# hellojialee/Improved-Body-Parts

Hardware: NVIDIA H100
Metric: grouping images/sec @128x128 heatmaps, 30 persons/img (higher is better)
Workload: dtype f32 body-part maps, f32 keypoint maps; f64 coordinates/scores

## Files before the change

improved_body_parts_b200/csrc/common.cuh:

```cuda
#pragma once

#include <cuda_runtime.h>
#include <stdint.h>

#include <algorithm>

namespace spg {

#ifdef SPG_TRACE
constexpr int kTraceCtas = 64, kTraceSlots = 1024;
__device__ unsigned long long g_spg_trace[kTraceCtas * kTraceSlots];
__device__ __forceinline__ void trace_put(int slot, int dep, bool value_only) {
    if (blockIdx.x < kTraceCtas && (threadIdx.x & 31) == 0) {
        unsigned long long t;
        asm volatile("mov.u64 %0, %%clock64;" : "=l"(t) : "r"(dep) : "memory");
        g_spg_trace[blockIdx.x * kTraceSlots + slot] = value_only ? (unsigned long long)(unsigned)dep : t;
    }
}
#define SPG_TR(slot, dep) ::spg::trace_put((slot), (int)(dep), false)
#define SPG_TRV(slot, v) ::spg::trace_put((slot), (int)(v), true)
#else
#define SPG_TR(slot, dep) do {} while (0)
#define SPG_TRV(slot, v) do {} while (0)
#endif

constexpr int kMaxParts = 32;
constexpr int kMaxLimbs = 64;
constexpr int kMaxCapPeaks = 128;
constexpr int kMaxCapRows = 128;
constexpr int kMaxRefineRadius = 4;
constexpr int kMaxOutJoints = 32;

constexpr uint32_t kStPeakOverflow = 1u << 0;
constexpr uint32_t kStCandOverflow = 1u << 1;
constexpr uint32_t kStRowOverflow = 1u << 2;
constexpr uint32_t kStSampleIndex = 1u << 3;
constexpr uint32_t kStAssert = 1u << 4;
constexpr uint32_t kStWireOverflow = 1u << 5;

struct Params {
    double thre1, thre2, connect_ration, len_rate, connection_tole, min_mean_score;
    int32_t mid_num, offset_radius, remove_recon, min_parts;
    int32_t crit1_strict, refresh_len_check;
};

struct Workspace {
    int K, L, J, capP, capC, capR, max_batch;
    int16_t limbs[kMaxLimbs * 2];
    int16_t out_from_part[kMaxOutJoints];
    double *peak_x, *peak_y;
    float *peak_score;
    uint32_t *peak_anchor;
    int32_t *peak_count;
    double *cand_prio, *cand_score;
    uint32_t *cand_ij;
    unsigned long long *cand_key;
    int32_t *cand_count;
    int32_t *surv_count;
    uint32_t *conn_ij;
    double *conn_score, *conn_norm;
    int32_t *conn_count;
    double *subset;
    int32_t *n_persons;
    double *people_xy;
    double *people_score;
    uint32_t *status;
    unsigned char *wire;
    long long wire_first;
    int wire_rows;
};

__device__ __forceinline__ uint32_t smem_u32(const void *p) { return (uint32_t)__cvta_generic_to_shared(p); }

__device__ __forceinline__ void mbar_init(uint64_t *bar, uint32_t count) {
    asm volatile("mbarrier.init.shared::cta.b64 [%0], %1;" ::"r"(smem_u32(bar)), "r"(count) : "memory");
}
__device__ __forceinline__ void fence_mbar_init() { asm volatile("fence.mbarrier_init.release.cluster;" ::: "memory"); }
__device__ __forceinline__ void fence_proxy_async() { asm volatile("fence.proxy.async.shared::cta;" ::: "memory"); }
__device__ __forceinline__ void mbar_expect_tx(uint64_t *bar, uint32_t bytes) {
    asm volatile("mbarrier.arrive.expect_tx.shared::cta.b64 _, [%0], %1;" ::"r"(smem_u32(bar)), "r"(bytes) : "memory");
}
__device__ __forceinline__ void bulk_g2s(void *dst_smem, const void *src_gmem, uint32_t bytes, uint64_t *bar) {
    asm volatile("cp.async.bulk.shared::cluster.global.mbarrier::complete_tx::bytes [%0], [%1], %2, [%3];" ::"r"(
                     smem_u32(dst_smem)),
                 "l"(src_gmem), "r"(bytes), "r"(smem_u32(bar))
                 : "memory");
}
__device__ __forceinline__ void mbar_arrive(uint64_t *bar) {
    asm volatile("mbarrier.arrive.shared::cta.b64 _, [%0];" ::"r"(smem_u32(bar)) : "memory");
}
__device__ __forceinline__ bool mbar_try_wait(uint64_t *bar, uint32_t parity) {
    uint32_t ok;
    asm volatile(
        "{\n"
        " .reg .pred p;\n"
        " mbarrier.try_wait.parity.shared::cta.b64 p, [%1], %2;\n"
        " selp.u32 %0, 1, 0, p;\n"
        "}\n"
        : "=r"(ok)
        : "r"(smem_u32(bar)), "r"(parity)
        : "memory");
    return ok != 0;
}
__device__ __forceinline__ void mbar_wait(uint64_t *bar, uint32_t parity) {
    while (!mbar_try_wait(bar, parity)) {
    }
}
__device__ __forceinline__ void mbar_wait_sleep(uint64_t *bar, uint32_t parity, uint32_t hint_ns = 20000u) {
    uint32_t ok = 0;
    while (!ok) {
        asm volatile(
            "{\n"
            " .reg .pred p;\n"
            " mbarrier.try_wait.parity.shared::cta.b64 p, [%1], %2, %3;\n"
            " selp.u32 %0, 1, 0, p;\n"
            "}\n"
            : "=r"(ok)
            : "r"(smem_u32(bar)), "r"(parity), "r"(hint_ns)
            : "memory");
    }
}

template <typename T>
__device__ __forceinline__ T pairwise_sum(const T *a, int n) {
    if (n < 8) {
        T res = (T)0;
        for (int i = 0; i < n; i++) res = res + a[i];
        return res;
    }
    T r[8];
#pragma unroll
    for (int k = 0; k < 8; k++) r[k] = a[k];
    int i = 8;
    for (; i < n - (n % 8); i += 8) {
#pragma unroll
        for (int k = 0; k < 8; k++) r[k] = r[k] + a[i + k];
    }
    T res = ((r[0] + r[1]) + (r[2] + r[3])) + ((r[4] + r[5]) + (r[6] + r[7]));
    for (; i < n; i++) res = res + a[i];
    return res;
}

}
```

improved_body_parts_b200/csrc/limb_score.cuh:

```cuda
#pragma once

#include "common.cuh"

namespace spg {

struct ScoreArgs {
    const void *paf;
    int64_t img_stride, chan_stride;
    int H, W, image_base, mid_num, screen;
    int crit1_strict;
    int exact_warps;
    double image_extent, thre2, connect_ration;
    Workspace ws;
};

constexpr int kScoreThreads = 512;
constexpr uint32_t kBulkChunkBytes = 32768;
constexpr int kScreenMaxMid = 63;
#ifndef SPG_SCREEN_SAMPLES
#define SPG_SCREEN_SAMPLES 10
#endif
constexpr int kScreenSamples = SPG_SCREEN_SAMPLES;
constexpr int kScreenMaxDim = 2048;

struct alignas(8) ScreenTab {
    float inv;
    signed char maxfail;
    unsigned char qn;
    unsigned char pad[2];
};

__host__ __device__ constexpr size_t screen_tables_bytes() {
    return (((size_t)(kScreenMaxMid + 1) * (sizeof(double) + sizeof(ScreenTab) + kScreenSamples * sizeof(float))) + 15) & ~(size_t)15;
}

__device__ __forceinline__ void build_screen_row(const ScoreArgs &a, int m, double *rcp, ScreenTab *tab, float *ts) {
    const double need = __dmul_rn(a.connect_ration, (double)m);
    int need_i = (int)need;
    if ((double)need_i < need || (a.crit1_strict && (double)need_i == need)) need_i++;
    rcp[m] = m > 0 ? __ddiv_rn(1.0, (double)m) : 0.0;
    const int lo = m / 8, hi = m - 1 - lo;
    const int qn = max(0, min(kScreenSamples, hi - lo + 1));
    for (int q = 0; q < kScreenSamples; q++)
        ts[m * kScreenSamples + q] = (float)(qn > 1 ? lo + (min(q, qn - 1) * (hi - lo)) / (qn - 1) : lo);
    ScreenTab t;
    t.inv = m > 1 ? 1.0f / (float)(m - 1) : 0.0f;
    t.maxfail = (signed char)max(min(m - need_i, 127), -1);
    t.qn = (unsigned char)qn;
    t.pad[0] = t.pad[1] = 0;
    tab[m] = t;
}

inline size_t score_smem_bytes(size_t plane_bytes, int capP) {
    const size_t plane = (plane_bytes + 127) & ~(size_t)127;
    const size_t peaks = (size_t)capP * (4 * sizeof(double) + 6 * sizeof(float) + 2);
    const size_t words = ((size_t)capP * capP + 31) / 32;
    return plane + ((peaks + 15) & ~(size_t)15) + screen_tables_bytes() + words * (sizeof(uint32_t) + sizeof(uint16_t)) + 16;
}

__device__ __forceinline__ bool inside_map(double x, double y, int H, int W) {
    return x >= 0.0 && x <= (double)(W - 1) && y >= 0.0 && y <= (double)(H - 1);
}

struct PairGeom {
    const double *ax, *ay, *bx, *by;
    const float *as, *bs;
    const double *rcp;
};

template <typename T, int kExactBatch = 1, typename TA = T>
__device__ __forceinline__ bool score_pair_exact(const T *__restrict__ plane, int H, int W, const ScoreArgs &a,
                                                 const PairGeom &g, int i, int j, bool interior, TA thre2,
                                                 double &score, double &prio, bool &bad) {
    const double ax = g.ax[i], ay = g.ay[i], bx = g.bx[j], by = g.by[j];
    const double vx = __dsub_rn(bx, ax), vy = __dsub_rn(by, ay);
    const double n2 = __dadd_rn(__dmul_rn(vx, vx), __dmul_rn(vy, vy));
    if (n2 == 0.0) return false;
    const double half = __dmul_rn(0.5, a.image_extent);
    const double Md = (double)a.mid_num;
    double norm = 0.0;
    int m = a.mid_num;
    const bool need_norm = n2 < __dmul_rn(Md, Md) || n2 > __dmul_rn(__dmul_rn(half, half), 1.0 - 1e-9);
    if (need_norm) {
        norm = __dsqrt_rn(n2);
        m = min(__double2int_rn(__dadd_rn(norm, 1.0)), a.mid_num);
    }
    double stepx = 0.0, stepy = 0.0;
    if (m > 1) {
        const double dd = (double)(m - 1);
        if (m - 1 <= kScreenMaxMid) {
            const double y = g.rcp[m - 1];
            const double qx = __dmul_rn(vx, y), qy = __dmul_rn(vy, y);
            stepx = __fma_rn(__fma_rn(-qx, dd, vx), y, qx);
            stepy = __fma_rn(__fma_rn(-qy, dd, vy), y, qy);
        } else {
            stepx = __ddiv_rn(vx, dd);
            stepy = __ddiv_rn(vy, dd);
        }
    }
    TA sum = (TA)0;
    int above = 0;
    if (interior) {
        const int last = m - 1;
        double td = 0.0;
        if constexpr (kExactBatch <= 1) {
#pragma unroll 4
            for (int t = 0; t < last; t++) {
                const int xi = __double2loint(__dadd_rn(__dadd_rn(__dmul_rn(td, stepx), ax), 6755399441055744.0));
                const int yi = __double2loint(__dadd_rn(__dadd_rn(__dmul_rn(td, stepy), ay), 6755399441055744.0));
                const TA v = (TA)plane[yi * W + xi];
                sum = sum + v;
                above += v > thre2;
                td = __dadd_rn(td, 1.0);
            }
        } else {
            for (int t0 = 0; t0 < last; t0 += kExactBatch) {
                T vv[kExactBatch > 0 ? kExactBatch : 1];
#pragma unroll
                for (int u = 0; u < kExactBatch; u++) {
                    const double tdu = t0 + u < last ? __dadd_rn(td, (double)u) : 0.0;
                    const int xi = __double2loint(__dadd_rn(__dadd_rn(__dmul_rn(tdu, stepx), ax), 6755399441055744.0));
                    const int yi = __double2loint(__dadd_rn(__dadd_rn(__dmul_rn(tdu, stepy), ay), 6755399441055744.0));
                    vv[u] = plane[yi * W + xi];
                }
#pragma unroll
                for (int u = 0; u < kExactBatch; u++) {
                    if (t0 + u < last) {
                        sum = sum + (TA)vv[u];
                        above += (TA)vv[u] > thre2;
                    }
                }
                td = __dadd_rn(td, (double)kExactBatch);
            }
        }
        const TA v = (TA)(m > 1 ? plane[__double2int_rn(by) * W + __double2int_rn(bx)]
                               : plane[__double2int_rn(ay) * W + __double2int_rn(ax)]);
        sum = sum + v;
        above += v > thre2;
    } else {
        for (int t = 0; t < m; t++) {
            double sx, sy;
            if (t == m - 1 && m > 1) {
                sx = bx;
                sy = by;
            } else {
                sx = __dadd_rn(__dmul_rn((double)t, stepx), ax);
                sy = __dadd_rn(__dmul_rn((double)t, stepy), ay);
            }
            int yi = __double2int_rn(sy), xi = __double2int_rn(sx);
            if (yi < 0) yi += H;
            if (xi < 0) xi += W;
            if (yi < 0 || yi >= H || xi < 0 || xi >= W) {
                bad = true;
                return false;
            }
            const TA v = (TA)plane[(size_t)yi * W + xi];
            sum = sum + v;
            above += v > thre2;
        }
    }
    double prior = 0.0;
    if (need_norm && norm > half) prior = __dsub_rn(__ddiv_rn(half, norm), 1.0);
    if (sizeof(TA) == 4) {
        float s = __fdiv_rn((float)sum, (float)m);
        s = __fadd_rn(s, prior < 0.0 ? __double2float_rn(prior) : 0.0f);
        const float pr = __fadd_rn(__fadd_rn(__fmul_rn(0.5f, s), __fmul_rn(0.25f, g.as[i])), __fmul_rn(0.25f, g.bs[j]));
        score = (double)s;
        prio = (double)pr;
    } else {
        score = __dadd_rn(__ddiv_rn((double)sum, (double)m), prior < 0.0 ? prior : 0.0);
        prio = __dadd_rn(__dadd_rn(__dmul_rn(0.5, score), (double)__fmul_rn(0.25f, g.as[i])),
                         (double)__fmul_rn(0.25f, g.bs[j]));
    }
    const double need = __dmul_rn(a.connect_ration, (double)m);
    const bool crit1 = a.crit1_strict ? (double)above > need : (double)above >= need;
    const bool crit2 = score > 0.0;
    return crit1 && crit2;
}

template <typename TA>
__device__ __forceinline__ void store_candidate(const Workspace &ws, size_t out_base, int pos, int i, int j, double score, double prio) {
    const uint32_t ij = ((uint32_t)i << 16) | (uint32_t)j;
    ws.cand_prio[out_base + pos] = prio;
    ws.cand_score[out_base + pos] = score;
    ws.cand_ij[out_base + pos] = ij;
    if (sizeof(TA) == 4) {
        const uint32_t b = __float_as_uint((float)prio);
        const uint32_t ord = (b & 0x80000000u) ? ~b : (b | 0x80000000u);
        ws.cand_key[out_base + pos] = ((unsigned long long)ord << 32) | (unsigned long long)(~ij);
    }
}

__device__ __forceinline__ void publish_limb(const Workspace &ws, int n, size_t slot, int ncand, int nsurv, uint32_t flags) {
    ws.cand_count[slot] = min(ncand, ws.capC);
    if (ws.surv_count) ws.surv_count[slot] = nsurv;
    if (ncand > ws.capC) flags |= kStCandOverflow;
    if (flags) atomicOr(&ws.status[n], flags);
}

__host__ __device__ inline float f32_not_above(double t) {
    float f = (float)t;
    if ((double)f > t) f = nextafterf(f, -INFINITY);
    return f;
}

template <typename T, bool STAGE, typename TA = T>
__global__ void __launch_bounds__(kScoreThreads, 3) limb_score_kernel(ScoreArgs a) {
    extern __shared__ __align__(128) unsigned char smem_raw[];
    __shared__ uint64_t bar;
    __shared__ int s_count;
    __shared__ uint32_t s_flags;
    __shared__ int s_total_surv;
    __shared__ uint32_t s_magic;

    const Workspace &ws = a.ws;
    const int tid = threadIdx.x, lane = tid & 31, warp = tid >> 5;
    const int k = blockIdx.x % ws.L;
    const int n_local = blockIdx.x / ws.L;
    const int n = a.image_base + n_local;
    const int H = a.H, W = a.W, capP = ws.capP;
    const T *gplane = reinterpret_cast<const T *>(a.paf) + (int64_t)n_local * a.img_stride + (int64_t)k * a.chan_stride;
    const size_t plane_bytes = (size_t)H * W * sizeof(T);
    if (tid == 0) {
        s_count = 0;
        s_flags = 0;
        if (STAGE) {
            mbar_init(&bar, 1);
            fence_mbar_init();
            mbar_expect_tx(&bar, (uint32_t)plane_bytes);
            for (size_t off = 0; off < plane_bytes; off += kBulkChunkBytes) {
                const uint32_t bytes = (uint32_t)min((size_t)kBulkChunkBytes, plane_bytes - off);
                bulk_g2s(smem_raw + off, reinterpret_cast<const unsigned char *>(gplane) + off, bytes, &bar);
            }
        }
    }
    const int pa = ws.limbs[2 * k], pb = ws.limbs[2 * k + 1];
    const int nA = min(ws.peak_count[(size_t)n * ws.K + pa], capP);
    const int nB = min(ws.peak_count[(size_t)n * ws.K + pb], capP);
    const size_t slot = (size_t)n * ws.L + k;
    if (nA == 0 || nB == 0) {
        if (tid == 0) {
            ws.cand_count[slot] = -1;
            if (STAGE) mbar_wait(&bar, 0);
        }
        return;
    }

    unsigned char *after = smem_raw + (STAGE ? ((plane_bytes + 127) & ~(size_t)127) : 0);
    double *s_ax = reinterpret_cast<double *>(after);
    double *s_ay = s_ax + capP;
    double *s_bx = s_ay + capP;
    double *s_by = s_bx + capP;
    float *s_as = reinterpret_cast<float *>(s_by + capP);
    float *s_bs = s_as + capP;
    float *s_fax = s_bs + capP;
    float *s_fay = s_fax + capP;
    float *s_fbx = s_fay + capP;
    float *s_fby = s_fbx + capP;
    unsigned char *s_ain = reinterpret_cast<unsigned char *>(s_fby + capP);
    unsigned char *s_bin = s_ain + capP;
    const size_t peaks_bytes = ((size_t)capP * (4 * sizeof(double) + 6 * sizeof(float) + 2) + 15) & ~(size_t)15;
    double *s_rcp = reinterpret_cast<double *>(after + peaks_bytes);
    ScreenTab *s_tab = reinterpret_cast<ScreenTab *>(s_rcp + (kScreenMaxMid + 1));
    float *s_ts = reinterpret_cast<float *>(s_tab + (kScreenMaxMid + 1));
    uint32_t *s_mask = reinterpret_cast<uint32_t *>(after + peaks_bytes + screen_tables_bytes());
    const int npairs = nA * nB;
    const int nwords = (npairs + 31) >> 5;
    uint16_t *s_prefix = reinterpret_cast<uint16_t *>(s_mask + (((size_t)capP * capP + 31) >> 5));

    const size_t baseA = ((size_t)n * ws.K + pa) * capP, baseB = ((size_t)n * ws.K + pb) * capP;
    const bool screen = a.screen && a.mid_num <= kScreenMaxMid && H <= kScreenMaxDim && W <= kScreenMaxDim;
    if (warp == 0) {
        for (int i = lane; i < nA; i += 32) {
            const double x = ws.peak_x[baseA + i], y = ws.peak_y[baseA + i];
            s_ax[i] = x; s_ay[i] = y;
            s_fax[i] = (float)(x * 64.0); s_fay[i] = (float)(y * 64.0);
            s_as[i] = ws.peak_score[baseA + i];
            s_ain[i] = inside_map(x, y, H, W);
        }
    } else if (warp == 1) {
        for (int j = lane; j < nB; j += 32) {
            const double x = ws.peak_x[baseB + j], y = ws.peak_y[baseB + j];
            s_bx[j] = x; s_by[j] = y;
            s_fbx[j] = (float)(x * 64.0); s_fby[j] = (float)(y * 64.0);
            s_bs[j] = ws.peak_score[baseB + j];
            s_bin[j] = inside_map(x, y, H, W);
        }
    } else if (warp < 4) {
        const int m = tid - 64;
        if (m <= a.mid_num && m <= kScreenMaxMid) build_screen_row(a, m, s_rcp, s_tab, s_ts);
        if (tid == 64 + 63) s_magic = nB > 1 ? 0xffffffffu / (uint32_t)nB + 1u : 0u;
    }
    __syncthreads();
    if (STAGE) mbar_wait(&bar, 0);
    const T *plane = STAGE ? reinterpret_cast<const T *>(smem_raw) : gplane;
    const T thre2 = (sizeof(T) == 4 && sizeof(TA) == 8) ? (T)f32_not_above(a.thre2) : (T)a.thre2;
    const TA thre2_exact = (TA)a.thre2;

    const uint32_t magic = s_magic;
    for (int base = 0; base < npairs; base += kScoreThreads) {
        const int p = base + tid;
        bool keep = false;
        if (p < npairs) {
            keep = true;
            if (screen) {
                const int i = nB > 1 ? (int)__umulhi((uint32_t)p, magic) : p;
                const int j = p - i * nB;
                if (s_ain[i] && s_bin[j]) {
                    const float ax64 = s_fax[i], ay64 = s_fay[i];
                    const float dx64 = s_fbx[j] - ax64, dy64 = s_fby[j] - ay64;
                    const float n2 = (dx64 * dx64 + dy64 * dy64) * (1.0f / 4096.0f);
                    if (n2 > 1e-6f) {
                        const float q = n2 * rsqrtf(n2) + 1.0f;
                        const float r = rintf(q);
                        const bool longp = q >= (float)a.mid_num + 0.51f;
                        int m = longp ? a.mid_num : min((int)r, a.mid_num);
                        if (!longp && !(fabsf(q - r) < 0.49f)) m = -1;
                        asm volatile("" : "+r"(m));
                        if (m >= 1) {
                            const ScreenTab tb = s_tab[m];
                            const int maxfail = tb.maxfail;
                            const int qn = tb.qn;
                            const float inv = tb.inv;
                            const float sx64 = dx64 * inv, sy64 = dy64 * inv;
                            const float *ts = s_ts + m * kScreenSamples;
                            int fails = 0;
                            for (int q2 = 0; q2 < qn; q2++) {
                                const float tf = ts[q2];
                                const int xs = __float2int_rn(__fmaf_rn(tf, sx64, ax64));
                                const int ys = __float2int_rn(__fmaf_rn(tf, sy64, ay64));
                                const unsigned cx = (unsigned)(xs + 33) & 63u, cy = (unsigned)(ys + 33) & 63u;
                                const T v = plane[((ys + 32) >> 6) * W + ((xs + 32) >> 6)];
                                fails += (min(cx, cy) > 2u) && !(v > thre2);
                            }
                            keep = fails <= maxfail;
                        }
                    }
                }
            }
        }
        const uint32_t bits = __ballot_sync(0xffffffffu, keep);
        if (lane == 0 && (base >> 5) + warp < nwords) s_mask[(base >> 5) + warp] = bits;
    }
    __syncthreads();
    if (warp == 0) {
        int running = 0;
        for (int w0 = 0; w0 < nwords; w0 += 32) {
            const int w = w0 + lane;
            const int c = w < nwords ? __popc(s_mask[w]) : 0;
            int incl = c;
#pragma unroll
            for (int d = 1; d < 32; d <<= 1) {
                const int o = __shfl_up_sync(0xffffffffu, incl, d);
                if (lane >= d) incl += o;
            }
            if (w < nwords) s_prefix[w] = (uint16_t)(running + incl - c);
            running += __shfl_sync(0xffffffffu, incl, 31);
        }
        if (lane == 0) s_total_surv = running;
    }
    __syncthreads();

    const int total_surv = s_total_surv;
    PairGeom g{s_ax, s_ay, s_bx, s_by, s_as, s_bs, s_rcp};
    const size_t out_base = slot * ws.capC;
    for (int sidx = tid; sidx < total_surv; sidx += kScoreThreads) {
        int lo = 0, hi = nwords - 1;
        while (lo < hi) {
            const int mid = (lo + hi + 1) >> 1;
            if ((int)s_prefix[mid] <= sidx) lo = mid; else hi = mid - 1;
        }
        const int bit = __fns(s_mask[lo], 0, sidx - (int)s_prefix[lo] + 1);
        const int p = (lo << 5) + bit;
        const int i = nB > 1 ? (int)__umulhi((uint32_t)p, magic) : p;
        const int j = p - i * nB;
        double score, prio;
        bool bad = false;
        const bool ok = score_pair_exact<T, 1, TA>(plane, H, W, a, g, i, j, s_ain[i] && s_bin[j], thre2_exact, score, prio, bad);
        if (bad) atomicOr(&s_flags, kStSampleIndex);
        if (ok) {
            const int pos = atomicAdd(&s_count, 1);
            if (pos < ws.capC) store_candidate<TA>(ws, out_base, pos, i, j, score, prio);
        }
    }
    __syncthreads();
    if (tid == 0) publish_limb(ws, n, slot, s_count, total_surv, s_flags);
}

}
```

improved_body_parts_b200/csrc/limb_score_persist.cuh:

```cuda
#pragma once

#include "limb_score.cuh"

namespace spg {

constexpr int kPersistThreads = 1024;
constexpr int kPersistSlots = 3;
constexpr int kMetaSlots = 5;
constexpr int kWorkerWarps = kPersistThreads / 32 - 1;
constexpr int kPersistMaxCapP = 64;
constexpr int kScreenTailBypass = 4;
constexpr int kPersistListCap = 1024;

struct PersistHdr {
    int nA, nB, npairs, n, k, special;
    uint32_t magic;
    int pad;
};

struct alignas(16) PeakSlot {
    double ax[kPersistMaxCapP], ay[kPersistMaxCapP], bx[kPersistMaxCapP], by[kPersistMaxCapP];
    float as[kPersistMaxCapP], bs[kPersistMaxCapP];
    float2 fa[kPersistMaxCapP], fb[kPersistMaxCapP];
    unsigned char ain[kPersistMaxCapP], bin[kPersistMaxCapP];
};

struct alignas(16) MetaSlot {
    PeakSlot peaks;
    uint16_t list[kPersistListCap];
    PersistHdr hdr;
    int nsurv, ncand, bnext;
    uint32_t flags;
};

constexpr size_t kPersistPlaneOffset = (screen_tables_bytes() + kMetaSlots * sizeof(MetaSlot) + 127) & ~(size_t)127;
inline size_t persist_smem_bytes(size_t plane_bytes, int ) {
    const size_t plane = (plane_bytes + 127) & ~(size_t)127;
    return kPersistPlaneOffset + kPersistSlots * plane + 128;
}

constexpr uint32_t kScreenBias = 0x4B400000u >> 6;

struct ScreenCtx {
    const PeakSlot *ps;
    uint32_t base;
    const ScreenTab *tab;
    const float *ts;
    int W, mid_num, nB;
    uint32_t magic;
    float thre2;
};

__device__ __forceinline__ void screen_pair(const ScreenCtx &c, int pc, bool valid, int &fails, int &qn, int &maxfail) {
    const int i = c.nB > 1 ? (int)__umulhi((uint32_t)pc, c.magic) : pc;
    const int jj = pc - i * c.nB;
    const float2 fa = c.ps->fa[i], fb = c.ps->fb[jj];
    const float dx64 = fb.x - fa.x, dy64 = fb.y - fa.y;
    const float n2 = (dx64 * dx64 + dy64 * dy64) * (1.0f / 4096.0f);
    float rs;
    asm("rsqrt.approx.ftz.f32 %0, %1;" : "=f"(rs) : "f"(n2));
    const float qf = n2 * rs + 1.0f;
    const float r = rintf(qf);
    const bool longp = qf >= (float)c.mid_num + 0.51f;
    int m = longp ? c.mid_num : min((int)r, c.mid_num);
    if (!longp && !(fabsf(qf - r) < 0.49f)) m = 0;
    if (!(n2 > 1e-6f) || !valid || fminf(fa.x, fb.x) < 0.0f) m = 0;
    m = max(m, 0);
    const ScreenTab tb = c.tab[m];
    qn = tb.qn;
    maxfail = tb.maxfail;
    const float sx64 = dx64 * tb.inv, sy64 = dy64 * tb.inv;
    const float ax64o = fa.x + 33.0f, ay64o = fa.y + 33.0f;
    const float *ts = c.ts + m * kScreenSamples;
    const int qmax = __reduce_max_sync(0xffffffffu, qn);
    const uint32_t base = c.base;
    fails = 0;
    auto sample = [&](int q2) {
        const float tf = ts[q2];
        const uint32_t xb = __float_as_uint(__fadd_rn(__fmaf_rn(tf, sx64, ax64o), 12582912.0f));
        const uint32_t yb = __float_as_uint(__fadd_rn(__fmaf_rn(tf, sy64, ay64o), 12582912.0f));
        float v;
        asm("ld.shared.f32 %0, [%1];" : "=f"(v) : "r"(base + 4u * ((yb >> 6) * (uint32_t)c.W + (xb >> 6))));
        fails += (int)(min(xb & 63u, yb & 63u) > 2u) & (int)!(v > c.thre2);
    };
    if (qmax == kScreenSamples) {
#pragma unroll
        for (int q2 = 0; q2 < kScreenSamples; q2++) sample(q2);
    } else {
#pragma unroll
        for (int q2 = 0; q2 < kScreenSamples; q2++) {
            if (q2 >= qmax) break;
            sample(q2);
        }
    }
    maxfail += qmax - qn;
}

template <typename TA>
__global__ void __launch_bounds__(kPersistThreads, 1) limb_score_persist_kernel(ScoreArgs a, int n_items) {
    extern __shared__ __align__(128) unsigned char smem_raw[];
    __shared__ uint64_t bar_full[kPersistSlots], bar_screened[kMetaSlots], bar_mfree[kMetaSlots];
    __shared__ uint32_t s_bias_bytes;

    using T = float;
    const Workspace &ws = a.ws;
    const int tid = threadIdx.x, lane = tid & 31, warp = tid >> 5;
    const int H = a.H, W = a.W, capP = ws.capP, L = ws.L;
    const size_t plane_bytes = (size_t)H * W * sizeof(T);
    const size_t plane_stride = (plane_bytes + 127) & ~(size_t)127;
    double *s_rcp = reinterpret_cast<double *>(smem_raw);
    ScreenTab *s_tab = reinterpret_cast<ScreenTab *>(s_rcp + (kScreenMaxMid + 1));
    float *s_ts = reinterpret_cast<float *>(s_tab + (kScreenMaxMid + 1));
    MetaSlot *s_meta = reinterpret_cast<MetaSlot *>(smem_raw + screen_tables_bytes());
    unsigned char *s_planes = smem_raw + kPersistPlaneOffset;
    const int nE = min(max(a.exact_warps, 1), kWorkerWarps - 1), nS = kWorkerWarps - nE;

    if (tid == 0) {
        for (int s = 0; s < kPersistSlots; s++) {
            mbar_init(&bar_full[s], 2);
        }
        for (int e = 0; e < kMetaSlots; e++) {
            mbar_init(&bar_screened[e], nS);
            mbar_init(&bar_mfree[e], nE);
            s_meta[e].nsurv = 0; s_meta[e].ncand = 0; s_meta[e].bnext = 0; s_meta[e].flags = 0;
        }
        s_bias_bytes = 4u * kScreenBias * (uint32_t)(W + 1);
        fence_mbar_init();
    }
    if (tid >= 32 && tid < 32 + kScreenMaxMid + 1) build_screen_row(a, tid - 32, s_rcp, s_tab, s_ts);
    __syncthreads();

    const int G = gridDim.x;
    const int nj = ((int)blockIdx.x < n_items) ? (n_items - 1 - (int)blockIdx.x) / G + 1 : 0;
    const bool screen = a.screen && a.mid_num <= kScreenMaxMid && H <= kScreenMaxDim && W <= kScreenMaxDim;
    const T thre2 = sizeof(TA) == 8 ? f32_not_above(a.thre2) : (T)a.thre2;
    const TA thre2_exact = (TA)a.thre2;
    auto plane_of = [&](int n_local, int k) {
        return reinterpret_cast<const T *>(a.paf) + (int64_t)n_local * a.img_stride + (int64_t)k * a.chan_stride;
    };

    if (warp == 0) {
        constexpr int kMaxE = kPersistMaxCapP / 32;
        double r_xa[kMaxE], r_ya[kMaxE], r_xb[kMaxE], r_yb[kMaxE];
        float r_sa[kMaxE], r_sb[kMaxE];
        int r_cntA = 0, r_cntB = 0;
        auto fetch = [&](int j) {
            const int item = (int)blockIdx.x + j * G;
            const int n_local = item / L, k = item - n_local * L;
            const int n = a.image_base + n_local;
            const int pa = ws.limbs[2 * k], pb = ws.limbs[2 * k + 1];
            r_cntA = ws.peak_count[(size_t)n * ws.K + pa];
            r_cntB = ws.peak_count[(size_t)n * ws.K + pb];
            const size_t baseA = ((size_t)n * ws.K + pa) * capP, baseB = ((size_t)n * ws.K + pb) * capP;
#pragma unroll
            for (int u = 0; u < kMaxE; u++) {
                const int e = lane + 32 * u;
                if (e < capP) {
                    r_xa[u] = ws.peak_x[baseA + e]; r_ya[u] = ws.peak_y[baseA + e];
                    r_xb[u] = ws.peak_x[baseB + e]; r_yb[u] = ws.peak_y[baseB + e];
                    r_sa[u] = ws.peak_score[baseA + e]; r_sb[u] = ws.peak_score[baseB + e];
                }
            }
        };
        auto close_item = [&](int jp) {
            if (lane == 0) {
                MetaSlot &ms = s_meta[jp % kMetaSlots];
                publish_limb(ws, ms.hdr.n, (size_t)ms.hdr.n * L + ms.hdr.k, ms.hdr.special ? -1 : ms.ncand, ms.nsurv, ms.flags);
                ms.nsurv = 0; ms.ncand = 0; ms.bnext = 0; ms.flags = 0;
            }
            __syncwarp();
        };
        if (nj > 0) fetch(0);
        for (int j = 0; j < nj; j++) {
            const int s = j % kPersistSlots, e = j % kMetaSlots;
            if (j >= kPersistSlots) {
                const int jp = j - kPersistSlots;
                mbar_wait_sleep(&bar_screened[jp % kMetaSlots], (jp / kMetaSlots) & 1);
            }
            const int item = (int)blockIdx.x + j * G;
            const int n_local = item / L, k = item - n_local * L;
            const int n = a.image_base + n_local;
            if (lane == 0) {
                const unsigned char *gplane = reinterpret_cast<const unsigned char *>(plane_of(n_local, k));
                unsigned char *dst = s_planes + s * plane_stride;
                mbar_expect_tx(&bar_full[s], (uint32_t)plane_bytes);
                for (size_t off = 0; off < plane_bytes; off += kBulkChunkBytes) {
                    const uint32_t bytes = (uint32_t)min((size_t)kBulkChunkBytes, plane_bytes - off);
                    bulk_g2s(dst + off, gplane + off, bytes, &bar_full[s]);
                }
            }
            if (j >= kMetaSlots) {
                mbar_wait_sleep(&bar_mfree[e], ((j / kMetaSlots) - 1) & 1);
                close_item(j - kMetaSlots);
            }
            MetaSlot &ms = s_meta[e];
            PeakSlot &ps = ms.peaks;
#pragma unroll
            for (int u = 0; u < kMaxE; u++) {
                const int q = lane + 32 * u;
                if (q < capP) {
                    const double xa = r_xa[u], ya = r_ya[u], xb = r_xb[u], yb = r_yb[u];
                    ps.ax[q] = xa; ps.ay[q] = ya; ps.bx[q] = xb; ps.by[q] = yb;
                    ps.as[q] = r_sa[u]; ps.bs[q] = r_sb[u];
                    const bool ain = inside_map(xa, ya, H, W), bin = inside_map(xb, yb, H, W);
                    ps.fa[q] = ain ? make_float2((float)(xa * 64.0), (float)(ya * 64.0)) : make_float2(-1.0f, 0.0f);
                    ps.fb[q] = bin ? make_float2((float)(xb * 64.0), (float)(yb * 64.0)) : make_float2(-1.0f, 0.0f);
                    ps.ain[q] = ain;
                    ps.bin[q] = bin;
                }
            }
            const int nA = min(r_cntA, capP), nB = min(r_cntB, capP);
            const bool special = nA == 0 || nB == 0;
            if (lane == 0) {
                PersistHdr h;
                h.nA = nA; h.nB = nB; h.npairs = special ? 0 : nA * nB; h.n = n; h.k = k; h.special = special;
                h.magic = nB > 1 ? 0xffffffffu / (uint32_t)nB + 1u : 0u;
                h.pad = 0;
                ms.hdr = h;
            }
            __syncwarp();
            if (lane == 0) mbar_arrive(&bar_full[s]);
            if (j + 1 < nj) fetch(j + 1);
        }
        for (int jp = max(0, nj - kMetaSlots); jp < nj; jp++) {
            mbar_wait_sleep(&bar_mfree[jp % kMetaSlots], (jp / kMetaSlots) & 1);
            close_item(jp);
        }
    } else {
        auto exact_one = [&](MetaSlot &ms, const T *plane, int p) {
            const PersistHdr &h = ms.hdr;
            const PeakSlot &ps = ms.peaks;
            const int nB = h.nB;
            const int i = nB > 1 ? (int)__umulhi((uint32_t)p, h.magic) : p;
            const int jj = p - i * nB;
            PairGeom g{ps.ax, ps.ay, ps.bx, ps.by, ps.as, ps.bs, s_rcp};
            double score, prio;
            bool bad = false;
            const bool ok = score_pair_exact<T, 10, TA>(plane, H, W, a, g, i, jj, ps.ain[i] && ps.bin[jj], thre2_exact, score, prio, bad);
            if (bad) atomicOr(&ms.flags, kStSampleIndex);
            if (ok) {
                const size_t out_base = ((size_t)h.n * L + h.k) * ws.capC;
                const int pos = atomicAdd(&ms.ncand, 1);
                if (pos < ws.capC) store_candidate<TA>(ws, out_base, pos, i, jj, score, prio);
            }
        };

        if (warp <= nS) {
            int c0 = warp - 1;
            for (int j = 0; j < nj; j++) {
                const int s = j % kPersistSlots, e = j % kMetaSlots;
                mbar_wait_sleep(&bar_full[s], (j / kPersistSlots) & 1);
                MetaSlot &ms = s_meta[e];
                const int npairs = ms.hdr.npairs;
                if (c0 * 32 < npairs) {
                    const T *plane = reinterpret_cast<const T *>(s_planes + s * plane_stride);
                    const ScreenCtx sc{&ms.peaks, smem_u32(plane) - *(volatile uint32_t *)&s_bias_bytes, s_tab, s_ts, W, a.mid_num,
                                       ms.hdr.nB, ms.hdr.magic, thre2};
                    for (int c = c0; c * 32 < npairs; c += nS) {
                        const int p = c * 32 + lane;
                        bool keep = p < npairs;
                        if (screen && npairs - c * 32 > kScreenTailBypass) {
                            int fails, qn, maxfail;
                            screen_pair(sc, min(p, npairs - 1), keep, fails, qn, maxfail);
                            if (qn > 0) keep = fails <= maxfail;
                        }
                        const uint32_t km = __ballot_sync(0xffffffffu, keep);
                        if (km) {
                            int at = 0;
                            if (lane == 0) at = atomicAdd(&ms.nsurv, __popc(km));
                            at = __shfl_sync(0xffffffffu, at, 0);
                            if (keep) {
                                const int at_me = at + __popc(km & ((1u << lane) - 1u));
                                if (at_me < kPersistListCap) ms.list[at_me] = (uint16_t)p;
                                else exact_one(ms, plane, p);
                            }
                        }
                    }
                }
                __syncwarp();
                if (lane == 0) mbar_arrive(&bar_screened[e]);
                if (++c0 == nS) c0 = 0;
            }
        } else {
            for (int j = 0; j < nj; j++) {
                const int e = j % kMetaSlots;
                mbar_wait_sleep(&bar_screened[e], (j / kMetaSlots) & 1);
                MetaSlot &ms = s_meta[e];
                const int ns = min(ms.nsurv, kPersistListCap);
                if (ns > 0) {
                    const T *gplane = plane_of(ms.hdr.n - a.image_base, ms.hdr.k);
                    for (;;) {
                        if (*(volatile int *)&ms.bnext * 32 >= ns) break;
                        int c = 0;
                        if (lane == 0) c = atomicAdd(&ms.bnext, 1);
                        c = __shfl_sync(0xffffffffu, c, 0);
                        if (c * 32 >= ns) break;
                        const int t = c * 32 + lane;
                        if (t < ns) exact_one(ms, gplane, ms.list[t]);
                        __syncwarp();
                    }
                }
                __syncwarp();
                if (lane == 0) mbar_arrive(&bar_mfree[e]);
            }
        }
    }
}

}
```

improved_body_parts_b200/csrc/spgroup.cu:

```cuda
#include "../../include/spgroup.h"

#include <cuda_runtime.h>

#include <algorithm>
#include <cstdarg>
#include <cstdio>
#include <cstdlib>
#include <cstring>
#include <new>
#include <string>
#include <vector>

#include "assemble.cuh"
#include "common.cuh"
#include "limb_match.cuh"
#include "limb_score.cuh"
#include "limb_score_persist.cuh"
#include "match_assemble.cuh"
#include "nms_peaks.cuh"
#include "nms_peaks_persist.cuh"
#include "nms_peaks_banded.cuh"
#include "postnet.cuh"

using namespace spg;

static_assert(sizeof(spg_params) == sizeof(spg::Params), "spg_params layout");

static thread_local std::string g_create_error;

struct spg_handle {
    spg_config cfg{};
    int device = 0;
    int sm_count = 0;
    size_t smem_optin = 0;
    Workspace ws{};
    std::vector<void *> allocs;
    void *in_heat = nullptr, *in_paf = nullptr;
    size_t in_heat_bytes = 0, in_paf_bytes = 0;
    unsigned int *done_counter = nullptr;
    unsigned long long *armed_flag = nullptr;
    unsigned long long armed_value = 0;
    double *heat_acc = nullptr;
    size_t heat_acc_elems = 0;
    cudaStream_t streams[2] = {nullptr, nullptr};
    int64_t launches = 0;
    const char *stage_kernel[5] = {"", "", "", "", ""};
    int persist = 1;
    int screen = 1;
    int exact_warps = 12;
    int ma_warps = kMAMatchWarps;
    int fuse_ma = 1;
    int cand_dtype = SPG_F32;
    int stage = 0;
    std::string err;
};

namespace {

int fail(spg_handle *h, int code, const char *fmt, ...) {
    char buf[512];
    va_list ap;
    va_start(ap, fmt);
    vsnprintf(buf, sizeof buf, fmt, ap);
    va_end(ap);
    if (h) h->err = buf; else g_create_error = buf;
    return code;
}

#define SPG_CUDA(h, call)                                                                              \
    do {                                                                                               \
        cudaError_t e_ = (call);                                                                       \
        if (e_ != cudaSuccess) return fail((h), SPG_E_CUDA, "%s failed: %s", #call, cudaGetErrorString(e_)); \
    } while (0)

template <typename T>
int dalloc(spg_handle *h, T **p, size_t count) {
    void *q = nullptr;
    SPG_CUDA(h, cudaMalloc(&q, std::max<size_t>(count, 1) * sizeof(T)));
    h->allocs.push_back(q);
    *p = static_cast<T *>(q);
    return SPG_OK;
}

struct DeviceGuard {
    int prev = -1;
    explicit DeviceGuard(int dev) {
        cudaGetDevice(&prev);
        if (prev != dev) cudaSetDevice(dev);
    }
    ~DeviceGuard() {
        int cur = -1;
        cudaGetDevice(&cur);
        if (prev >= 0 && cur != prev) cudaSetDevice(prev);
    }
};

int check_dims(spg_handle *h, int n, int H, int W) {
    if (n < 0 || n > h->cfg.max_batch) return fail(h, SPG_E_INVALID, "n_images %d outside [0, max_batch=%d]", n, h->cfg.max_batch);
    if (H < 2 || W < 2 || H > h->cfg.max_h || W > h->cfg.max_w || H > 32767 || W > 32767)
        return fail(h, SPG_E_INVALID, "map %dx%d outside [2, %dx%d]", H, W, h->cfg.max_h, h->cfg.max_w);
    return SPG_OK;
}

int check_params(spg_handle *h, const spg_params *p) {
    if (!p) return fail(h, SPG_E_INVALID, "params is NULL");
    if (p->offset_radius < 0 || p->offset_radius > kMaxRefineRadius)
        return fail(h, SPG_E_INVALID, "offset_radius %d outside [0, %d]", p->offset_radius, kMaxRefineRadius);
    if (p->mid_num < 1) return fail(h, SPG_E_INVALID, "mid_num must be >= 1");
    return SPG_OK;
}

int launch_nms(spg_handle *h, const float *heat, int64_t img_stride, int64_t chan_stride, int base, int n, int H, int W,
               const spg_params *p, cudaStream_t st) {
    if (n == 0) return SPG_OK;
    NmsArgs a{};
    a.heat = heat;
    a.img_stride = img_stride;
    a.chan_stride = chan_stride;
    a.H = H;
    a.W = W;
    a.radius = p->offset_radius;
    a.use_bulk = (W % 4 == 0) && (img_stride % 4 == 0) && (chan_stride % 4 == 0) && ((reinterpret_cast<uintptr_t>(heat) & 15) == 0);
    a.image_base = base;
    a.thr = (float)p->thre1;
    a.ws = h->ws;
    if (h->persist && a.use_bulk && nms_persist_smem_bytes(H, W, h->ws.capP) <= h->smem_optin && (size_t)H * W / 4 < 65536 &&
        (size_t)H * W * sizeof(float) < (1u << 20) &&
        ((size_t)H * W / 4 + kNmsPScanners - 1) / kNmsPScanners <= (size_t)32 * kNmsPMaxIter) {
        const size_t psm = nms_persist_smem_bytes(H, W, h->ws.capP);
        const int items = n * h->ws.K;
        SPG_CUDA(h, cudaFuncSetAttribute(nms_peaks_persist_kernel, cudaFuncAttributeMaxDynamicSharedMemorySize, (int)psm));
        nms_peaks_persist_kernel<<<std::min(items, h->sm_count), kNmsPThreads, psm, st>>>(a, items);
        h->stage_kernel[0] = "nms_peaks_persist_kernel";
        h->launches++;
        SPG_CUDA(h, cudaGetLastError());
        return SPG_OK;
    }
    const NmsBanding bg = (h->persist && a.use_bulk) ? nms_banding(H, W, h->ws.capP, h->smem_optin - 1024) : NmsBanding{};
    if (bg.slots >= kNmsBTeams) {
        const int items = n * h->ws.K;
        a.band_rows = bg.band_rows;
        SPG_CUDA(h, cudaFuncSetAttribute(nms_peaks_banded_kernel, cudaFuncAttributeMaxDynamicSharedMemorySize, (int)bg.smem));
        nms_peaks_banded_kernel<<<std::min(items, h->sm_count), kNmsPThreads, bg.smem, st>>>(a, items, bg.slots, bg.n_bands);
        h->stage_kernel[0] = "nms_peaks_banded_kernel";
        h->launches++;
        SPG_CUDA(h, cudaGetLastError());
        return SPG_OK;
    }
    a.band_rows = std::max(4, std::min(H, 4096 / W));
    const size_t smem = nms_smem_bytes(a.band_rows, H, W, h->ws.capP);
    if (smem > h->smem_optin) return fail(h, SPG_E_INVALID, "map width %d needs %zu B of shared memory per band", W, smem);
    SPG_CUDA(h, cudaFuncSetAttribute(nms_peaks_kernel, cudaFuncAttributeMaxDynamicSharedMemorySize, (int)smem));
    nms_peaks_kernel<<<n * h->ws.K, kNmsThreads, smem, st>>>(a);
    h->stage_kernel[0] = "nms_peaks_kernel";
    h->launches++;
    SPG_CUDA(h, cudaGetLastError());
    return SPG_OK;
}

template <typename T, typename TA = T>
int launch_score_t(spg_handle *h, const ScoreArgs &a, int n, cudaStream_t st) {
    const size_t plane_bytes = (size_t)a.H * a.W * sizeof(T);
    const size_t staged = score_smem_bytes(plane_bytes, h->ws.capP);
    const bool aligned = (plane_bytes % 16 == 0) && ((a.img_stride * sizeof(T)) % 16 == 0) && ((a.chan_stride * sizeof(T)) % 16 == 0) &&
                         ((reinterpret_cast<uintptr_t>(a.paf) & 15) == 0) && plane_bytes < (1u << 20);
    const int grid = n * h->ws.L;
    if (sizeof(T) == 4 && h->persist && aligned && h->ws.capP <= kPersistMaxCapP &&
        persist_smem_bytes(plane_bytes, h->ws.capP) <= h->smem_optin) {
        const size_t smem = persist_smem_bytes(plane_bytes, h->ws.capP);
        SPG_CUDA(h, cudaFuncSetAttribute(limb_score_persist_kernel<TA>, cudaFuncAttributeMaxDynamicSharedMemorySize, (int)smem));
        limb_score_persist_kernel<TA><<<std::min(grid, h->sm_count), kPersistThreads, smem, st>>>(a, grid);
        h->stage_kernel[1] = sizeof(TA) == 4 ? "limb_score_persist_kernel<float>" : "limb_score_persist_kernel<double>";
    } else if (aligned && staged <= h->smem_optin) {
        SPG_CUDA(h, (cudaFuncSetAttribute(limb_score_kernel<T, true, TA>, cudaFuncAttributeMaxDynamicSharedMemorySize, (int)staged)));
        limb_score_kernel<T, true, TA><<<grid, kScoreThreads, staged, st>>>(a);
        h->stage_kernel[1] = sizeof(T) == 8 ? "limb_score_kernel<double,true>" : sizeof(TA) == 4 ? "limb_score_kernel<float,true>" : "limb_score_kernel<float,true,double>";
    } else {
        const size_t smem = score_smem_bytes(0, h->ws.capP);
        limb_score_kernel<T, false, TA><<<grid, kScoreThreads, smem, st>>>(a);
        h->stage_kernel[1] = sizeof(T) == 8 ? "limb_score_kernel<double,false>" : sizeof(TA) == 4 ? "limb_score_kernel<float,false>" : "limb_score_kernel<float,false,double>";
    }
    h->launches++;
    SPG_CUDA(h, cudaGetLastError());
    return SPG_OK;
}

int launch_score(spg_handle *h, const void *paf, int dtype, int64_t img_stride, int64_t chan_stride, int base, int n, int H,
                 int W, double extent, const spg_params *p, cudaStream_t st) {
    if (n == 0) return SPG_OK;
    ScoreArgs a{};
    a.paf = paf;
    a.img_stride = img_stride;
    a.chan_stride = chan_stride;
    a.H = H;
    a.W = W;
    a.image_base = base;
    a.mid_num = p->mid_num;
    a.image_extent = extent;
    a.thre2 = p->thre2;
    a.connect_ration = p->connect_ration;
    a.screen = h->screen;
    a.crit1_strict = p->crit1_strict != 0;
    a.exact_warps = h->exact_warps;
    a.ws = h->ws;
    h->cand_dtype = dtype;
    if (dtype == SPG_F64) return launch_score_t<double>(h, a, n, st);
    if (dtype == SPG_F32_AS_F64) return launch_score_t<float, double>(h, a, n, st);
    return launch_score_t<float>(h, a, n, st);
}

int launch_match(spg_handle *h, int base, int n, cudaStream_t st) {
    if (n == 0) return SPG_OK;
    MatchArgs a{};
    a.n_images = n;
    a.image_base = base;
    a.keys_valid = h->cand_dtype == SPG_F32;
    a.ws = h->ws;
    const int warps = n * h->ws.L;
    const int blocks = (warps * 32 + kMatchThreads - 1) / kMatchThreads;
    limb_match_kernel<<<blocks, kMatchThreads, 0, st>>>(a);
    h->stage_kernel[2] = "limb_match_kernel";
    h->launches++;
    SPG_CUDA(h, cudaGetLastError());
    return SPG_OK;
}

AssembleArgs assemble_args(const spg_handle *h, int base, int n, const spg_params *p) {
    AssembleArgs a{};
    a.n_images = n;
    a.image_base = base;
    a.len_rate = p->len_rate;
    a.connection_tole = p->connection_tole;
    a.min_mean_score = p->min_mean_score;
    a.remove_recon = p->remove_recon;
    a.min_parts = p->min_parts;
    a.refresh_len_check = p->refresh_len_check != 0;
    a.wire_flag = h->armed_flag; a.wire_flag_value = h->armed_value; a.done_counter = h->done_counter;
    a.ws = h->ws;
    a.ws.wire_first += base;
    return a;
}

int launch_assemble(spg_handle *h, int base, int n, const spg_params *p, cudaStream_t st) {
    if (n == 0) return SPG_OK;
    AssembleArgs a = assemble_args(h, base, n, p);
    h->armed_flag = nullptr;
    a.use_bulk = ((size_t)h->ws.L * h->ws.capP * sizeof(uint32_t)) % 16 == 0;
    const size_t smem = assemble_smem_bytes(h->ws.K, h->ws.capP, h->ws.capR) + assemble_conn_bytes(h->ws.L, h->ws.capP);
    if (smem > h->smem_optin) return fail(h, SPG_E_INVALID, "capacities need %zu B of shared memory in assemble (limit %zu)", smem, h->smem_optin);
    SPG_CUDA(h, cudaFuncSetAttribute(assemble_kernel, cudaFuncAttributeMaxDynamicSharedMemorySize, (int)smem));
    assemble_kernel<<<n, kAssembleThreads, smem, st>>>(a);
    h->stage_kernel[3] = "assemble_kernel";
    h->launches++;
    SPG_CUDA(h, cudaGetLastError());
    return SPG_OK;
}

int launch_match_assemble(spg_handle *h, int base, int n, const spg_params *p, cudaStream_t st) {
    if (n == 0) return SPG_OK;
    AssembleArgs a = assemble_args(h, base, n, p);
    a.use_bulk = ((size_t)h->ws.K * h->ws.capP * sizeof(float)) % 16 == 0;
    const size_t smem = match_assemble_smem_bytes(h->ws.K, h->ws.L, h->ws.capP, h->ws.capR, h->ma_warps);
    if (smem > h->smem_optin) {
        int rc;
        if ((rc = launch_match(h, base, n, st))) return rc;
        return launch_assemble(h, base, n, p, st);
    }
    h->armed_flag = nullptr;
    SPG_CUDA(h, cudaFuncSetAttribute(match_assemble_kernel, cudaFuncAttributeMaxDynamicSharedMemorySize, (int)smem));
    match_assemble_kernel<<<n, 32 * (1 + h->ma_warps), smem, st>>>(a, h->cand_dtype == SPG_F32);
    h->stage_kernel[2] = "match_assemble_kernel";
    h->stage_kernel[3] = "";
    h->launches++;
    SPG_CUDA(h, cudaGetLastError());
    return SPG_OK;
}

int run_all(spg_handle *h, const float *heat, int64_t his, int64_t hcs, const void *paf, int dtype, int64_t pis, int64_t pcs,
            int base, int n, int H, int W, double extent, const spg_params *p, cudaStream_t st) {
    int rc;
    SPG_CUDA(h, cudaMemsetAsync(h->ws.status + base, 0, sizeof(uint32_t) * (size_t)n, st));
    if ((rc = launch_nms(h, heat, his, hcs, base, n, H, W, p, st))) return rc;
    if ((rc = launch_score(h, paf, dtype, pis, pcs, base, n, H, W, extent, p, st))) return rc;
    if (h->fuse_ma) return launch_match_assemble(h, base, n, p, st);
    if ((rc = launch_match(h, base, n, st))) return rc;
    if ((rc = launch_assemble(h, base, n, p, st))) return rc;
    return SPG_OK;
}

__global__ void wire_signal_kernel(unsigned long long *word, unsigned long long value) {
    __threadfence_system();
    asm volatile("st.release.sys.global.u64 [%0], %1;" ::"l"(word), "l"(value) : "memory");
}

struct WireWords {
    unsigned long long *p[32];
    int n;
};
__global__ void wire_signal_many_kernel(WireWords w, unsigned long long value) {
    __threadfence_system();
    if ((int)threadIdx.x < w.n) asm volatile("st.release.sys.global.u64 [%0], %1;" ::"l"(w.p[threadIdx.x]), "l"(value) : "memory");
}

__global__ void wire_wait_kernel(const unsigned long long *word, unsigned long long value) {
    unsigned long long v;
    do {
        asm volatile("ld.acquire.sys.global.u64 %0, [%1];" : "=l"(v) : "l"(word) : "memory");
        if (v < value) __nanosleep(500);
    } while (v < value);
}

}

extern "C" {

#ifdef SPG_TRACE
int spg_trace_read(unsigned long long *out, size_t n_words, int clear) {
    const size_t n = std::min(n_words, (size_t)spg::kTraceCtas * spg::kTraceSlots);
    if (cudaMemcpyFromSymbol(out, spg::g_spg_trace, n * sizeof(unsigned long long)) != cudaSuccess) return -1;
    if (clear) {
        void *p = nullptr;
        if (cudaGetSymbolAddress(&p, spg::g_spg_trace) != cudaSuccess) return -1;
        if (cudaMemset(p, 0, sizeof(spg::g_spg_trace)) != cudaSuccess) return -1;
    }
    return 0;
}
#endif

int spg_abi_version(void) { return SPG_ABI_VERSION; }

const char *spg_last_error(const spg_handle *h) { return h ? h->err.c_str() : g_create_error.c_str(); }

int spg_create(const spg_config *cfg, spg_handle **out) {
    if (!cfg || !out) return fail(nullptr, SPG_E_INVALID, "cfg/out is NULL");
    *out = nullptr;
    if (cfg->abi_version != SPG_ABI_VERSION) return fail(nullptr, SPG_E_INVALID, "ABI version %d != %d", cfg->abi_version, SPG_ABI_VERSION);
    if (cfg->n_parts < 1 || cfg->n_parts > kMaxParts || cfg->n_limbs < 1 || cfg->n_limbs > kMaxLimbs || !cfg->limbs)
        return fail(nullptr, SPG_E_INVALID, "n_parts in [1,%d], n_limbs in [1,%d], limbs non-NULL required", kMaxParts, kMaxLimbs);
    if (cfg->n_out_joints < 0 || cfg->n_out_joints > kMaxOutJoints || (cfg->n_out_joints && !cfg->out_from_part))
        return fail(nullptr, SPG_E_INVALID, "n_out_joints in [0,%d]", kMaxOutJoints);
    if (cfg->max_peaks_per_part < 1 || cfg->max_peaks_per_part > kMaxCapPeaks)
        return fail(nullptr, SPG_E_INVALID, "max_peaks_per_part in [1,%d]", kMaxCapPeaks);
    if (cfg->max_person_rows < 1 || cfg->max_person_rows > kMaxCapRows)
        return fail(nullptr, SPG_E_INVALID, "max_person_rows in [1,%d]", kMaxCapRows);
    if (cfg->max_cands_per_limb < 1 || cfg->max_batch < 1 || cfg->max_h < 2 || cfg->max_w < 2)
        return fail(nullptr, SPG_E_INVALID, "max_cands_per_limb, max_batch >= 1 and max_h, max_w >= 2 required");
    for (int k = 0; k < cfg->n_limbs * 2; k++)
        if (cfg->limbs[k] < 0 || cfg->limbs[k] >= cfg->n_parts) return fail(nullptr, SPG_E_INVALID, "limb table entry %d out of range", k);
    for (int g = 0; g < cfg->n_out_joints; g++)
        if (cfg->out_from_part[g] < 0 || cfg->out_from_part[g] >= cfg->n_parts) return fail(nullptr, SPG_E_INVALID, "out_from_part[%d] out of range", g);

    int ndev = 0;
// ... 615 lines not shown
```

Baseline: 567,900.

## Spread screen samples across limb in persistent scorer and raise exact warps

The persistent limb scorer now builds its screening sample table so the first six samples are spread evenly across the limb's sample range, with the remaining samples filling the unused positions. The goal is to make early-rejection screening find failing candidates sooner, so fewer pairs need exact scoring. The default number of exact-scoring warps also goes from 12 to 14. The change also adds compile-time trace instrumentation (first/last atomic timestamps per item), which is inactive by default. The reordering changes which samples are checked first, so screening still has to produce the same outcomes.

```diff
diff --git a/improved_body_parts_b200/csrc/common.cuh b/improved_body_parts_b200/csrc/common.cuh
--- a/improved_body_parts_b200/csrc/common.cuh
+++ b/improved_body_parts_b200/csrc/common.cuh
@@ -10,18 +10,25 @@
 #ifdef SPG_TRACE
 constexpr int kTraceCtas = 64, kTraceSlots = 1024;
 __device__ unsigned long long g_spg_trace[kTraceCtas * kTraceSlots];
-__device__ __forceinline__ void trace_put(int slot, int dep, bool value_only) {
+__device__ __forceinline__ void trace_put(int slot, int dep, int mode) {
     if (blockIdx.x < kTraceCtas && (threadIdx.x & 31) == 0) {
         unsigned long long t;
         asm volatile("mov.u64 %0, %%clock64;" : "=l"(t) : "r"(dep) : "memory");
-        g_spg_trace[blockIdx.x * kTraceSlots + slot] = value_only ? (unsigned long long)(unsigned)dep : t;
+        unsigned long long *w = &g_spg_trace[blockIdx.x * kTraceSlots + slot];
+        if (mode == 2) atomicCAS(w, 0ull, t);
+        else if (mode == 3) atomicMax(w, t);
+        else *w = mode == 1 ? (unsigned long long)(unsigned)dep : t;
     }
 }
-#define SPG_TR(slot, dep) ::spg::trace_put((slot), (int)(dep), false)
-#define SPG_TRV(slot, v) ::spg::trace_put((slot), (int)(v), true)
+#define SPG_TR(slot, dep) ::spg::trace_put((slot), (int)(dep), 0)
+#define SPG_TRV(slot, v) ::spg::trace_put((slot), (int)(v), 1)
+#define SPG_TR_FIRST(slot, dep) ::spg::trace_put((slot), (int)(dep), 2)
+#define SPG_TR_LAST(slot, dep) ::spg::trace_put((slot), (int)(dep), 3)
 #else
 #define SPG_TR(slot, dep) do {} while (0)
 #define SPG_TRV(slot, v) do {} while (0)
+#define SPG_TR_FIRST(slot, dep) do {} while (0)
+#define SPG_TR_LAST(slot, dep) do {} while (0)
 #endif
 
 constexpr int kMaxParts = 32;
diff --git a/improved_body_parts_b200/csrc/limb_score.cuh b/improved_body_parts_b200/csrc/limb_score.cuh
--- a/improved_body_parts_b200/csrc/limb_score.cuh
+++ b/improved_body_parts_b200/csrc/limb_score.cuh
@@ -22,6 +22,7 @@
 #endif
 constexpr int kScreenSamples = SPG_SCREEN_SAMPLES;
 constexpr int kScreenMaxDim = 2048;
+constexpr int kScreenSpreadFirst = kScreenSamples < 6 ? kScreenSamples : 6;
 
 struct alignas(8) ScreenTab {
     float inv;
@@ -34,15 +35,34 @@
     return (((size_t)(kScreenMaxMid + 1) * (sizeof(double) + sizeof(ScreenTab) + kScreenSamples * sizeof(float))) + 15) & ~(size_t)15;
 }
 
-__device__ __forceinline__ void build_screen_row(const ScoreArgs &a, int m, double *rcp, ScreenTab *tab, float *ts) {
+__device__ __forceinline__ void build_screen_row(const ScoreArgs &a, int m, double *rcp, ScreenTab *tab, float *ts, bool spread) {
     const double need = __dmul_rn(a.connect_ration, (double)m);
     int need_i = (int)need;
     if ((double)need_i < need || (a.crit1_strict && (double)need_i == need)) need_i++;
     rcp[m] = m > 0 ? __ddiv_rn(1.0, (double)m) : 0.0;
     const int lo = m / 8, hi = m - 1 - lo;
     const int qn = max(0, min(kScreenSamples, hi - lo + 1));
-    for (int q = 0; q < kScreenSamples; q++)
-        ts[m * kScreenSamples + q] = (float)(qn > 1 ? lo + (min(q, qn - 1) * (hi - lo)) / (qn - 1) : lo);
+    auto put = [&](int q, int r) { ts[m * kScreenSamples + q] = (float)(qn > 1 ? lo + (r * (hi - lo)) / (qn - 1) : lo); };
+    if (!spread) {
+        for (int q = 0; q < kScreenSamples; q++) put(q, min(q, max(qn - 1, 0)));
+    } else {
+        const int s1 = min(kScreenSpreadFirst, qn);
+        const float step = s1 > 1 ? (float)(qn - 1) / (float)(s1 - 1) : 0.0f;
+        uint32_t taken = 0;
+        for (int q = 0; q < s1; q++) {
+            const int r = min((int)__fadd_rn(__fmul_rn((float)q, step), 0.5f), qn - 1);
+            taken |= 1u << r;
+            put(q, r);
+        }
+        for (int q = s1, r = 0; q < kScreenSamples; q++) {
+            if (q < qn) {
+                while (taken >> r & 1u) r++;
+                put(q, r++);
+            } else {
+                put(q, max(qn - 1, 0));
+            }
+        }
+    }
     ScreenTab t;
     t.inv = m > 1 ? 1.0f / (float)(m - 1) : 0.0f;
     t.maxfail = (signed char)max(min(m - need_i, 127), -1);
@@ -288,7 +308,7 @@
         }
     } else if (warp < 4) {
         const int m = tid - 64;
-        if (m <= a.mid_num && m <= kScreenMaxMid) build_screen_row(a, m, s_rcp, s_tab, s_ts);
+        if (m <= a.mid_num && m <= kScreenMaxMid) build_screen_row(a, m, s_rcp, s_tab, s_ts, false);
         if (tid == 64 + 63) s_magic = nB > 1 ? 0xffffffffu / (uint32_t)nB + 1u : 0u;
     }
     __syncthreads();
diff --git a/improved_body_parts_b200/csrc/limb_score_persist.cuh b/improved_body_parts_b200/csrc/limb_score_persist.cuh
--- a/improved_body_parts_b200/csrc/limb_score_persist.cuh
+++ b/improved_body_parts_b200/csrc/limb_score_persist.cuh
@@ -11,6 +11,9 @@
 constexpr int kPersistMaxCapP = 64;
 constexpr int kScreenTailBypass = 4;
 constexpr int kPersistListCap = 1024;
+
+constexpr int kTrItemWords = 16, kTrItems = 64;
+#define SPG_TR_ITEM(kind, j, f, dep) do { if ((j) < kTrItems) kind(kTrItemWords * (j) + (f), dep); } while (0)
 
 struct PersistHdr {
     int nA, nB, npairs, n, k, special;
@@ -127,7 +130,7 @@
         s_bias_bytes = 4u * kScreenBias * (uint32_t)(W + 1);
         fence_mbar_init();
     }
-    if (tid >= 32 && tid < 32 + kScreenMaxMid + 1) build_screen_row(a, tid - 32, s_rcp, s_tab, s_ts);
+    if (tid >= 32 && tid < 32 + kScreenMaxMid + 1) build_screen_row(a, tid - 32, s_rcp, s_tab, s_ts, true);
     __syncthreads();
 
     const int G = gridDim.x;
@@ -165,6 +168,9 @@
         auto close_item = [&](int jp) {
             if (lane == 0) {
                 MetaSlot &ms = s_meta[jp % kMetaSlots];
+                SPG_TR_ITEM(SPG_TR, jp, 8, ms.nsurv);
+                SPG_TR_ITEM(SPG_TRV, jp, 9, ms.nsurv);
+                SPG_TR_ITEM(SPG_TRV, jp, 10, ms.ncand);
                 publish_limb(ws, ms.hdr.n, (size_t)ms.hdr.n * L + ms.hdr.k, ms.hdr.special ? -1 : ms.ncand, ms.nsurv, ms.flags);
                 ms.nsurv = 0; ms.ncand = 0; ms.bnext = 0; ms.flags = 0;
             }
@@ -173,6 +179,7 @@
         if (nj > 0) fetch(0);
         for (int j = 0; j < nj; j++) {
             const int s = j % kPersistSlots, e = j % kMetaSlots;
+            SPG_TR_ITEM(SPG_TR, j, 0, j);
             if (j >= kPersistSlots) {
                 const int jp = j - kPersistSlots;
                 mbar_wait_sleep(&bar_screened[jp % kMetaSlots], (jp / kMetaSlots) & 1);
@@ -189,8 +196,11 @@
                     bulk_g2s(dst + off, gplane + off, bytes, &bar_full[s]);
                 }
             }
+            SPG_TR_ITEM(SPG_TR, j, 1, j);
             if (j >= kMetaSlots) {
+                SPG_TR_ITEM(SPG_TR, j, 2, j);
                 mbar_wait_sleep(&bar_mfree[e], ((j / kMetaSlots) - 1) & 1);
+                SPG_TR_ITEM(SPG_TR, j, 3, j);
                 close_item(j - kMetaSlots);
             }
             MetaSlot &ms = s_meta[e];
@@ -219,6 +229,7 @@
                 ms.hdr = h;
             }
             __syncwarp();
+            SPG_TR_ITEM(SPG_TR, j, 4, j);
             if (lane == 0) mbar_arrive(&bar_full[s]);
             if (j + 1 < nj) fetch(j + 1);
         }
@@ -250,6 +261,7 @@
             for (int j = 0; j < nj; j++) {
                 const int s = j % kPersistSlots, e = j % kMetaSlots;
                 mbar_wait_sleep(&bar_full[s], (j / kPersistSlots) & 1);
+                SPG_TR_ITEM(SPG_TR_FIRST, j, 5, j);
                 MetaSlot &ms = s_meta[e];
                 const int npairs = ms.hdr.npairs;
                 if (c0 * 32 < npairs) {
@@ -278,6 +290,8 @@
                     }
                 }
                 __syncwarp();
+                SPG_TR_ITEM(SPG_TR_FIRST, j, 6, j);
+                SPG_TR_ITEM(SPG_TR_LAST, j, 7, j);
                 if (lane == 0) mbar_arrive(&bar_screened[e]);
                 if (++c0 == nS) c0 = 0;
             }
@@ -301,6 +315,7 @@
                     }
                 }
                 __syncwarp();
+                SPG_TR_ITEM(SPG_TR_LAST, j, 11, j);
                 if (lane == 0) mbar_arrive(&bar_mfree[e]);
             }
         }
diff --git a/improved_body_parts_b200/csrc/spgroup.cu b/improved_body_parts_b200/csrc/spgroup.cu
--- a/improved_body_parts_b200/csrc/spgroup.cu
+++ b/improved_body_parts_b200/csrc/spgroup.cu
@@ -47,7 +47,7 @@
     const char *stage_kernel[5] = {"", "", "", "", ""};
     int persist = 1;
     int screen = 1;
-    int exact_warps = 12;
+    int exact_warps = 14;
     int ma_warps = kMAMatchWarps;
     int fuse_ma = 1;
     int cand_dtype = SPG_F32;
```

After: 591,300 (median of 6 runs). 4.1% higher.
